# tachitachi/SR-WaveNet

Measured on AMD Instinct MI355X. Metric: audio samples/sec (fwd+bwd) 30-layer teacher WaveNet, higher is better.
Workload: dtype bf16; 1 GPU; 30-layer teacher WaveNet (3x[1..512] dilations, 64 res / 256 skip ch, 256-way mu-law softmax), fwd+bwd+Adam, batch 8x16000 samples per GPU; global_batch=8, seq_len=16000, parallelism=dp1, launch=hipGraph

## Files before the change

sr-wavenet_amd/build.py:

```python
from __future__ import annotations

import os
import subprocess
import sys
from concurrent.futures import ThreadPoolExecutor

HERE = os.path.dirname(os.path.abspath(__file__))
CSRC = os.path.join(HERE, "csrc")
LIB = os.path.join(HERE, "libsrwn.so")
MANIFEST = os.path.join(HERE, "libsrwn.manifest.json")
IO_LIB = os.path.join(HERE, "libsrwn_io.so")
PYB_SRC = os.path.join(CSRC, "srwn_pybind.cpp")
PYB_NAME = "_srwn_pyb"
IO_SOURCES = ["srwn_tfrecord.cpp"]
CXX = os.environ.get("CXX", "g++")
SOURCES = ["srwn_util.hip", "srwn_fwd.hip", "srwn_bwd.hip", "srwn_opt.hip", "srwn_pool.hip", "srwn_gemm.hip", "srwn_wgrad2.hip", "srwn_gen.hip", "srwn_gen16.hip", "srwn_flow.hip", "srwn_enc.hip", "srwn_nc.hip", "srwn_ncstream.hip", "srwn_group.hip", "srwn_wgradt.hip", "srwn_ops.hip", "srwn_head.hip", "srwn_siamese.hip", "srwn_wngate.hip", "srwn_stream.hip", "srwn_recog.hip", "srwn_score.hip", "srwn_embed.hip", "srwn_flow_inv.hip", "srwn_data.hip", "srwn_draw.hip", "srwn_augment.hip", "srwn_resample.hip", "srwn_room.hip", "srwn_eval.hip", "srwn_pair_eval.hip"]
HIPCC = os.environ.get("HIPCC", "/opt/rocm/bin/hipcc")
FLAGS = ["--offload-arch=gfx950", "-O3", "-fPIC", "-std=c++17", "-Wno-pass-failed", "-ffp-contract=on"]
NO_SPILL = {"srwn_wgradt.hip": ["wgrad_skip_wt_kernel"], "srwn_siamese.hip": ["contrastive_head_kernel"],
            "srwn_wngate.hip": ["wavenet_layer_fwd_kernel", "wavenet_layer_bwd_kernel"],
            "srwn_ncstream.hip": ["nc_encode_frames_kernel", "nc_encode_frames_kernelINS_10NcListArgs"],
            "srwn_recog.hip": ["pooled_stream_head_kernel"], "srwn_score.hip": ["stream_score_head_kernel"],
            "srwn_embed.hip": ["window_embed_match_kernel", "gallery_match_kernel"],
            "srwn_pair_eval.hip": ["embed_collect_kernel", "pair_sweep_kernel"],
            "srwn_room.hip": ["batch_draw_room_kernel", "pair_draw_room_kernel"]}


def _deps():
    hdrs = [os.path.join(CSRC, f) for f in os.listdir(CSRC) if f.endswith(".h")]
    hdrs.append(os.path.join(HERE, "..", "include", "srwn.h"))
    return hdrs


def source_hashes():
    import hashlib
    files = [os.path.join(CSRC, f) for f in sorted(os.listdir(CSRC)) if f.endswith((".hip", ".h", ".cpp"))]
    files.append(os.path.join(HERE, "..", "include", "srwn.h"))
    files.append(os.path.join(HERE, "..", "include", "srwn_io.h"))
    out = {}
    for f in files:
        if os.path.exists(f):
            out[os.path.relpath(f, os.path.join(HERE, ".."))] = hashlib.sha256(open(f, "rb").read()).hexdigest()
    return out


def _stale(target, srcs):
    if not os.path.exists(target):
        return True
    t = os.path.getmtime(target)
    return any(os.path.getmtime(s) > t for s in srcs)


def _sha(paths, extra=""):
    import hashlib
    h = hashlib.sha256(extra.encode())
    for f in paths:
        h.update(open(f, "rb").read())
    return h.hexdigest()


def _check_no_spill(src, obj, remarks, kernels):
    import re
    seen = {}
    name = None
    for line in remarks.splitlines():
        m = re.search(r"Function Name: (\S+)", line)
        if m:
            name = m.group(1)
        m = re.search(r"(?:[VS]GPRs Spill|ScratchSize \[bytes/lane\]): (\d+)", line)
        if m and name:
            seen[name] = seen.get(name, 0) + int(m.group(1))
    for k in kernels:
        hit = [(n, v) for n, v in seen.items() if k in n]
        if not hit or any(v for _, v in hit):
            if os.path.exists(obj):
                os.remove(obj)
            raise RuntimeError("%s: kernel %s must not spill registers or use scratch: %s" % (src, k, hit or "not found"))


def _check_inflight(src, obj, flags, kernels):
    import importlib.util
    spec = importlib.util.spec_from_file_location("_srwn_asmcheck", os.path.join(HERE, "asmcheck.py"))
    ac = importlib.util.module_from_spec(spec)
    spec.loader.exec_module(ac)
    cmd = [HIPCC] + flags + ["--cuda-device-only", "-S", src, "-o", "-"]
    r = subprocess.run(cmd, capture_output=True, text=True)
    if r.returncode != 0:
        raise RuntimeError("hipcc -S failed for %s:\n%s" % (src, r.stderr[-4000:]))
    for k in kernels:
        bad = ac.check_inflight_loads(r.stdout, k)
        if bad:
            if os.path.exists(obj):
                os.remove(obj)
            raise RuntimeError("%s: kernel %s touches the destination of a load that may still be in flight:\n  %s"
                               % (src, k, "\n  ".join(bad[:8])))


def build(force: bool = False, verbose: bool = False, diag: bool = False, variant: str = "", extra_flags=()) -> str:
    import json
    per_src = {}
    for f in list(extra_flags):
        if ".hip:" in f:
            name, fl = f.split(":", 1)
            per_src.setdefault(name, []).extend(fl.split("=", 1) if fl.startswith("-mllvm=") else [fl])
    extra_flags = [f for f in extra_flags if ".hip:" not in f]
    flags = FLAGS + (["-DSRWN_DIAG"] if diag else []) + list(extra_flags)
    if variant:
        diag = True
# ... 132 lines not shown
```

sr-wavenet_amd/csrc/srwn_gemm.hip:

```cpp
#include <cstdlib>
#include "srwn_common.h"
#include "srwn_host.h"
#include "../../include/srwn.h"

using namespace srwn;

#define SRWN_EPI_SOFTMAX_CE 3

struct RgArgs {
  const void* x; int64_t x_row_stride; int64_t x_chunk_stride; int chunk_len; int ks_total;
  const void* wpack; const float* bias; void* y; int64_t y_row_stride; int cout_valid; int64_t rows;
  const void* aux; int64_t aux_row_stride;
  const int32_t* targets; float* loss_partials; float* logits_out; float grad_scale;
  int tap_T; int tap_step; const float* frame_add; int64_t frame_add_ld; int frames; int pool; float frame_add_scale;
  int safe_wait;
  unsigned long long* stamps;
};

#ifndef SRWN_RG_PIPE
#define SRWN_RG_PIPE 1
#endif
#ifndef SRWN_RG_PIPE_VALU
#define SRWN_RG_PIPE_VALU 6
#endif
constexpr bool kRgPipe = SRWN_RG_PIPE != 0;
constexpr int kRgPipeValu = SRWN_RG_PIPE_VALU;
template <bool STAMP> struct RgStamper {
  unsigned long long* p; int n;
  __device__ __forceinline__ void operator()(int tag) {
    if (STAMP && p && n < 512) { p[n] = ((unsigned long long)tag << 48) | (__builtin_amdgcn_s_memtime() & 0xffffffffffffull); ++n; }
  }
};

template <typename T> __device__ __forceinline__ void glds16(const void* g, void* l) {
  __builtin_amdgcn_global_load_lds((const __attribute__((address_space(1))) void*)g,
                                   (__attribute__((address_space(3))) void*)l, 16, 0, 0);
}

__device__ __forceinline__ void glds16_untracked(const void* g, unsigned lds_addr) {
  unsigned keep;
  asm volatile("s_mov_b32 %0, m0\n\ts_mov_b32 m0, %2\n\ts_nop 0\n\tglobal_load_lds_dwordx4 %1, off\n\ts_mov_b32 m0, %0"
               : "=&s"(keep) : "v"(g), "s"(lds_addr) : "memory");
}

constexpr int rg_waves(int epi, int nt) { return (epi == SRWN_EPI_SOFTMAX_CE || nt == 2) ? 4 : 8; }

template <typename T, int MT, int KSC, int PRO, int EPI, int NT, bool TAPS = false, bool STAMP = false>
__global__ __launch_bounds__(64 * rg_waves(EPI, NT), (EPI == SRWN_EPI_SOFTMAX_CE || NT == 2) ? 1 : 2) void rowgemm_kernel(RgArgs a) {
  constexpr int kRgWaves = rg_waves(EPI, NT);
  RgStamper<STAMP> stamp{nullptr, 0};
  if (STAMP && blockIdx.x == 0 && (threadIdx.x & 63) == 0 && ((threadIdx.x >> 6) & 3) == 0) stamp.p = a.stamps + (threadIdx.x >> 8) * 512;
  stamp(1);
  static_assert(MT % 2 == 0, "outputs are emitted in 64-channel groups");
  static_assert(EPI != SRWN_EPI_SOFTMAX_CE || NT == 1, "softmax epilogue holds one column tile");
  constexpr int FB = sizeof(Frag<T>) * 64;
  constexpr int CHUNK_B = MT * KSC * FB;
  constexpr int PIECES = CHUNK_B / 1024;
  static_assert(PIECES % kRgWaves == 0, "chunk must split evenly over the waves");
  extern __shared__ __attribute__((aligned(16))) char smem[];

  const int lane = threadIdx.x & 63;
  const int wave = __builtin_amdgcn_readfirstlane(threadIdx.x >> 6);
  const int col = lane & 31, half = lane >> 5;
  const int64_t tile0 = ((int64_t)blockIdx.x * kRgWaves + wave) * NT;
  int64_t rowv[NT];
  bool valid[NT];
  int tclip[NT];
#pragma unroll
  for (int nt = 0; nt < NT; ++nt) {
    rowv[nt] = (tile0 + nt) * 32 + col;
    valid[nt] = rowv[nt] < a.rows;
    tclip[nt] = TAPS ? (int)((valid[nt] ? rowv[nt] : (a.rows - 1)) % a.tap_T) : 0;
  }
  const int nchunks = a.ks_total / KSC;
  const char* wbase = reinterpret_cast<const char*>(a.wpack);
  const unsigned lds_base = (unsigned)(size_t)(__attribute__((address_space(3))) char*)smem;

  auto stage = [&](int c, int buf) {
#pragma unroll
    for (int i = 0; i < PIECES / kRgWaves; ++i) {
      const int p = wave * (PIECES / kRgWaves) + i;
      const int mt = p / (KSC * FB / 1024), within = (p % (KSC * FB / 1024)) * 1024;
      const char* g = wbase + ((size_t)mt * a.ks_total + (size_t)c * KSC) * FB + within + lane * 16;
      const unsigned l = lds_base + (unsigned)(buf * CHUNK_B + mt * (KSC * FB) + within);
      glds16_untracked(g, __builtin_amdgcn_readfirstlane(l));
    }
  };
  int cur_chunk = 0, cur_within = 0, cur_next = 0;
  int64_t cur_off = 0;
  const int64_t chunk_step = a.x_chunk_stride - a.chunk_len + 16;
  auto cursor = [&](int (&chunk)[KSC], int (&within)[KSC], int64_t (&off)[KSC]) {
    int cc = cur_chunk, ww = cur_within;
    int64_t oo = cur_off;
#pragma unroll
    for (int ks = 0; ks < KSC; ++ks) {
      chunk[ks] = cc; within[ks] = ww; off[ks] = oo;
      const bool wrap = ww + 16 >= a.chunk_len;
      ww = wrap ? 0 : ww + 16;
      oo += wrap ? chunk_step : (int64_t)16;
      cc += wrap ? 1 : 0;
    }
    if (cur_next + 1 < nchunks) { cur_chunk = cc; cur_within = ww; cur_off = oo; ++cur_next; }
  };
  auto load_b = [&](Frag<T> (&dst)[NT][KSC], bool (&ok)[NT][KSC]) {
    int chunks[KSC], withins[KSC];
    int64_t offs[KSC];
    cursor(chunks, withins, offs);
#pragma unroll
    for (int nt = 0; nt < NT; ++nt)
#pragma unroll
      for (int ks = 0; ks < KSC; ++ks) {
        const int chunk = chunks[ks], within = withins[ks];
        const int64_t rbase = valid[nt] ? rowv[nt] : (a.rows - 1);
        if (TAPS) {
          const int tp = tclip[nt] + chunk * a.tap_step;
          ok[nt][ks] = tp >= 0 && tp < a.tap_T;
          const T* p = reinterpret_cast<const T*>(a.x) + (rbase + (ok[nt][ks] ? chunk * a.tap_step : 0)) * a.x_row_stride +
                       within + 8 * half;
          dst[nt][ks] = load_nat(p);
        } else {
          ok[nt][ks] = true;
          const T* p = reinterpret_cast<const T*>(a.x) + offs[ks] + rbase * a.x_row_stride + 8 * half;
          dst[nt][ks] = load_nat(p);
        }
      }
// ... 191 lines not shown
    float s = 0.0f;
    {
      const int cv = opaque(a.cout_valid);
#pragma unroll
      for (int mt = 0; mt < MT; ++mt)
#pragma unroll
        for (int q = 0; q < 16; ++q) {
          const int n = 32 * mt + crow(q, half);
          const float e = (n < cv) ? __expf(acc[mt][0][q] - m) : 0.0f;
          acc[mt][0][q] = e;
          s += e;
        }
    }
    s += __shfl_xor(s, 32);
    const float lse = m + __logf(s);
    float loss = (vld && half == 0) ? (lse - vt) : 0.0f;
#pragma unroll
    for (int off = 16; off > 0; off >>= 1) loss += __shfl_xor(loss, off);
    if (lane == 0 && tile0 * 32 < a.rows) a.loss_partials[tile0] = loss;
    if (a.y) {
      const float ps = a.grad_scale / s;
      const int64_t r0 = tile0 * 32;
      const int rows_valid = (a.rows - r0) < 32 ? (int)(a.rows - r0) : 32;
      T* ytile = reinterpret_cast<T*>(a.y) + (rows_valid > 0 ? r0 : 0) * a.y_row_stride;
#pragma unroll
      for (int j = 0; j < MT / 2; ++j) {
        const int tg = opaque(tgt);
        float v[2][16];
#pragma unroll
        for (int m2 = 0; m2 < 2; ++m2)
#pragma unroll
          for (int q = 0; q < 16; ++q) {
            const int n = 32 * (2 * j + m2) + crow(q, half);
            v[m2][q] = fmaf(acc[2 * j + m2][0][q], ps, n == tg ? -a.grad_scale : 0.0f);
          }
        store_rows_via_lds<T, 2>(rstage, ytile + 64 * j, a.y_row_stride, v, rows_valid, lane);
      }
    }
    return;
  }

#pragma unroll
  for (int nt = 0; nt < NT; ++nt) {
    const int64_t r0 = (tile0 + nt) * 32;
    const int rows_valid = (a.rows - r0) < 32 ? (int)(a.rows - r0) : 32;
    T* ytile = reinterpret_cast<T*>(a.y) + (rows_valid > 0 ? r0 : 0) * a.y_row_stride;
    const T* arow = (EPI == SRWN_EPI_MASK)
                        ? reinterpret_cast<const T*>(a.aux) + (valid[nt] ? rowv[nt] : 0) * a.aux_row_stride
                        : nullptr;
    const float* frow = nullptr;
    if (TAPS && a.frame_add) {
      const int64_t rr = valid[nt] ? rowv[nt] : 0;
      frow = a.frame_add + ((rr / a.tap_T) * a.frames + (tclip[nt] / a.pool)) * a.frame_add_ld;
    }
#pragma unroll
    for (int j = 0; j < MT / 2; ++j) {
      if (64 * j >= a.cout_valid) continue;
      float v[2][16];
#pragma unroll
      for (int m2 = 0; m2 < 2; ++m2)
#pragma unroll
        for (int g = 0; g < 4; ++g) {
          f32x4 mk = {1.f, 1.f, 1.f, 1.f};
          if (EPI == SRWN_EPI_MASK) mk = load4(arow + 32 * (2 * j + m2) + 8 * g + 4 * half);
          f32x4 fa = {0.f, 0.f, 0.f, 0.f};
          if (TAPS && frow) fa = *reinterpret_cast<const f32x4*>(frow + 32 * (2 * j + m2) + 8 * g + 4 * half);
#pragma unroll
          for (int e = 0; e < 4; ++e) {
            float x = acc[2 * j + m2][nt][4 * g + e];
            if (TAPS) x = fmaf(fa[e], a.frame_add_scale, x);
            if (EPI == SRWN_EPI_RELU) x = fmaxf(x, 0.0f);
            if (EPI == SRWN_EPI_MASK) x = (mk[e] > 0.0f) ? x : 0.0f;
            v[m2][4 * g + e] = x;
          }
        }
      store_rows_via_lds<T, 2>(rstage, ytile + 64 * j, a.y_row_stride, v, rows_valid, lane);
    }
  }
}

struct CgArgs {
  const void* x; int64_t x_row_stride; const void* wpack; void* y; int64_t y_layer_stride; int nlayers; int64_t rows;
  int safe_wait;
};

template <typename T, int RT, int KSS, int NBUF, int NW>
__global__ __launch_bounds__(64 * NW) void colgemm_kernel(CgArgs a) {
  constexpr int R = 32 * RT;
  constexpr int FB = sizeof(Frag<T>) * 64;
  constexpr int CHUNK_B = RT * KSS * FB;
  extern __shared__ __attribute__((aligned(16))) char smem[];
  const int lane = threadIdx.x & 63;
  const int wave = __builtin_amdgcn_readfirstlane(threadIdx.x >> 6);
  const int col = lane & 31, half = lane >> 5;
  T* stage = reinterpret_cast<T*>(smem + NBUF * CHUNK_B) + wave * (32 * RowStage<T>::stride(R));
  const int64_t row0 = ((int64_t)blockIdx.x * NW + wave) * 32;
  const int64_t row = row0 + col;
  const bool valid = row < a.rows;
  const int rows_valid = (a.rows - row0) < 32 ? (int)(a.rows - row0) : 32;
  const char* wbase = reinterpret_cast<const char*>(a.wpack);

  constexpr bool COUNTED = sizeof(T) == 2 && NBUF == 2;
  constexpr int PIECES = CHUNK_B / 1024;
  static_assert(!COUNTED || PIECES % NW == 0, "weight image must split evenly over the waves");
  const unsigned lds_base = (unsigned)(size_t)(__attribute__((address_space(3))) char*)smem;
  auto dma = [&](int l, int buf) __attribute__((always_inline)) {
#pragma unroll
    for (int i = 0; i < PIECES / NW; ++i) {
      const int p = wave * (PIECES / NW) + i;
      glds16_untracked(wbase + (size_t)l * CHUNK_B + (size_t)p * 1024 + lane * 16,
                       __builtin_amdgcn_readfirstlane(lds_base + (unsigned)(buf * CHUNK_B + p * 1024)));
    }
  };
  if constexpr (COUNTED) dma(0, 0); else lds_dma_copy(wbase, smem, CHUNK_B, wave, lane, NW);
  Frag<T> bf[KSS];
  {
    const T* p = reinterpret_cast<const T*>(a.x) + (valid ? row : 0) * a.x_row_stride + 8 * half;
#pragma unroll
    for (int ks = 0; ks < KSS; ++ks) bf[ks] = load_nat(p + 16 * ks);
#pragma unroll
    for (int ks = 0; ks < KSS; ++ks) bf[ks] = valid ? bf[ks] : zero_frag<T>();
  }
  if constexpr (COUNTED) asm volatile("s_waitcnt vmcnt(0)" ::: "memory");
  __syncthreads();
  for (int l = 0; l < a.nlayers; ++l) {
    const int buf = (NBUF == 2) ? (l & 1) : 0;
    if (NBUF == 2 && l + 1 < a.nlayers) {
      if constexpr (COUNTED) dma(l + 1, (l + 1) & 1);
      else lds_dma_copy(wbase + (size_t)(l + 1) * CHUNK_B, smem + ((l + 1) & 1) * CHUNK_B, CHUNK_B, wave, lane, NW);
    }
    const Frag<T>* lw = reinterpret_cast<const Frag<T>*>(smem + buf * CHUNK_B) + lane;
    f32x16 acc[RT];
#pragma unroll
    for (int mt = 0; mt < RT; ++mt)
#pragma unroll
      for (int q = 0; q < 16; ++q) acc[mt][q] = 0.0f;
    constexpr int G = 4;
    Frag<T> af[2][G][RT];
#pragma unroll
    for (int j = 0; j < G; ++j)
#pragma unroll
      for (int mt = 0; mt < RT; ++mt) af[0][j][mt] = lw[(mt * KSS + j) * 64];
#pragma unroll
    for (int k0 = 0; k0 < KSS; k0 += G) {
      if (k0 + G < KSS) {
#pragma unroll
        for (int j = 0; j < G; ++j)
#pragma unroll
          for (int mt = 0; mt < RT; ++mt) af[((k0 / G) + 1) & 1][j][mt] = lw[(mt * KSS + k0 + G + j) * 64];
      }
      __builtin_amdgcn_sched_barrier(0);
#pragma unroll
      for (int j = 0; j < G; ++j)
#pragma unroll
        for (int mt = 0; mt < RT; ++mt) mma(acc[mt], af[(k0 / G) & 1][j][mt], bf[k0 + j]);
      __builtin_amdgcn_sched_barrier(0);
    }
    float v[RT][16];
#pragma unroll
    for (int mt = 0; mt < RT; ++mt)
#pragma unroll
      for (int q = 0; q < 16; ++q) v[mt][q] = acc[mt][q];
    T* ytile = reinterpret_cast<T*>(a.y) + (int64_t)l * a.y_layer_stride + (rows_valid > 0 ? row0 : 0) * R;
    if constexpr (COUNTED) {
      constexpr int STORES = 32 / (64 / (R / RowStage<T>::VEC));
      if (rows_valid > 0) {
        store_rows_via_lds<T, RT, true>(stage, ytile, R, v, rows_valid, lane);
        if (a.safe_wait) asm volatile("s_waitcnt vmcnt(0)" ::: "memory");
        else asm volatile("s_waitcnt vmcnt(%0)" ::"n"(STORES) : "memory");
      } else {
        asm volatile("s_waitcnt vmcnt(0)" ::: "memory");
      }
      asm volatile("s_waitcnt lgkmcnt(0)\n\ts_barrier" ::: "memory");
    } else {
      store_rows_via_lds<T, RT>(stage, ytile, R, v, rows_valid, lane);
      __syncthreads();
    }
    if (NBUF == 1 && l + 1 < a.nlayers) {
      lds_dma_copy(wbase + (size_t)(l + 1) * CHUNK_B, smem, CHUNK_B, wave, lane, NW);
      __syncthreads();
    }
  }
}

template <typename T, int RT, int KSS, int NBUF>
static int launch_cg(const CgArgs& a, hipStream_t st) {
  constexpr int R = 32 * RT;
  constexpr int NW = (sizeof(T) == 2) ? 8 : 4;
  const size_t sh = (size_t)NBUF * RT * KSS * sizeof(Frag<T>) * 64 + (size_t)NW * 32 * RowStage<T>::stride(R) * sizeof(T);
  auto kfn = colgemm_kernel<T, RT, KSS, NBUF, NW>;
  hipError_t e = hipFuncSetAttribute((const void*)kfn, hipFuncAttributeMaxDynamicSharedMemorySize, (int)sh);
  if (e != hipSuccess) return set_error((int)e, "skip_dgrad_all: LDS %zu: %s", sh, hipGetErrorString(e));
  hipLaunchKernelGGL(kfn, dim3((unsigned)((a.rows + 32 * NW - 1) / (32 * NW))), dim3(64 * NW), sh, st, a);
  return check_launch("skip_dgrad_all");
}

extern "C" int srwn_skip_dgrad_all(const void* dtotal, const void* wskipT_all, void* dcs, int64_t dcs_layer_stride,
                                   int32_t nlayers, int64_t rows, int32_t R, int32_t S, int32_t dtype, void* stream) {
  if (rows == 0 || nlayers == 0) return 0;
  if (!dtotal || !wskipT_all || !dcs) return set_error(SRWN_E_NULL, "skip_dgrad_all: null pointer");
  if (rows < 0 || nlayers < 0) return set_error(SRWN_E_SHAPE, "skip_dgrad_all: rows=%lld layers=%d", (long long)rows, nlayers);
  CgArgs a{dtotal, S, wskipT_all, dcs, dcs_layer_stride, nlayers, rows, safe_wait()};
  hipStream_t st = (hipStream_t)stream;
  if (R == 64 && S == 256) {
    if (dtype == SRWN_BF16) return launch_cg<bf16_t, 2, 16, 2>(a, st);
    if (dtype == SRWN_F32) return launch_cg<float, 2, 16, 1>(a, st);
    return set_error(SRWN_E_DTYPE, "skip_dgrad_all: dtype %d", dtype);
  }
  if (R == 32 && S == 128) {
    if (dtype == SRWN_BF16) return launch_cg<bf16_t, 1, 8, 2>(a, st);
    if (dtype == SRWN_F32) return launch_cg<float, 1, 8, 2>(a, st);
    return set_error(SRWN_E_DTYPE, "skip_dgrad_all: dtype %d", dtype);
  }
  return set_error(SRWN_E_UNSUPPORTED, "skip_dgrad_all: built for (R,S) = (64,256) and (32,128), got (%d,%d)", R, S);
}

namespace srwn {

template <typename T, int MT, int KSC, int NT>
static int launch_rg(const RgArgs& a, int pro, int epi, hipStream_t st) {
  constexpr int CHUNK_B = MT * KSC * (int)sizeof(Frag<T>) * 64;
  constexpr int NTS = 1;
  const int nw = rg_waves(epi, (epi == SRWN_EPI_SOFTMAX_CE) ? NTS : NT);
  const size_t stage_b = (size_t)nw * 32 * RowStage<T>::stride(64) * sizeof(T);
  const size_t sh = 2 * (size_t)CHUNK_B > stage_b ? 2 * (size_t)CHUNK_B : stage_b;
  const int rows_per_block = 32 * nw * ((epi == SRWN_EPI_SOFTMAX_CE) ? NTS : NT);
  dim3 grid((unsigned)((a.rows + rows_per_block - 1) / rows_per_block)), block(64 * nw);
#define SRWN_RG(P, E)                                                                                        \
  if (pro == P && epi == E) {                                                                                \
    auto kfn = rowgemm_kernel<T, MT, KSC, P, E, (E == SRWN_EPI_SOFTMAX_CE) ? 1 : NT>;                        \
    if constexpr (sizeof(T) == 2 && P == SRWN_PRO_GATE && E == SRWN_EPI_RELU && NT == 1 && MT == 8) {         \
      SRWN_DIAG_ONLY(if (a.stamps) kfn = rowgemm_kernel<T, MT, KSC, P, E, NT, false, true>;)    \
    }                                                                                                        \
    if (sh > 32768) {                                                                                        \
      hipError_t e = hipFuncSetAttribute((const void*)kfn, hipFuncAttributeMaxDynamicSharedMemorySize, (int)sh); \
      if (e != hipSuccess) return set_error((int)e, "rowgemm: LDS %zu: %s", sh, hipGetErrorString(e));       \
    }                                                                                                        \
    hipLaunchKernelGGL(kfn, grid, block, sh, st, a);                                                         \
    return check_launch("rowgemm");                                                                          \
  }
  SRWN_RG(SRWN_PRO_NONE, SRWN_EPI_NONE)
  SRWN_RG(SRWN_PRO_NONE, SRWN_EPI_RELU)
  SRWN_RG(SRWN_PRO_NONE, SRWN_EPI_MASK)
  SRWN_RG(SRWN_PRO_GATE, SRWN_EPI_NONE)
  SRWN_RG(SRWN_PRO_GATE, SRWN_EPI_RELU)
  SRWN_RG(SRWN_PRO_NONE, SRWN_EPI_SOFTMAX_CE)
#undef SRWN_RG
  return set_error(SRWN_E_UNSUPPORTED, "rowgemm: pro %d / epi %d combination not built", pro, epi);
}

template <typename T, int MT, int KSC>
static int launch_rg_taps(const RgArgs& a, int epi, hipStream_t st) {
  constexpr int CHUNK_B = MT * KSC * (int)sizeof(Frag<T>) * 64;
  constexpr int kRgWaves = rg_waves(SRWN_EPI_NONE, 1);
  const size_t stage_b = (size_t)kRgWaves * 32 * RowStage<T>::stride(64) * sizeof(T);
  const size_t sh = 2 * (size_t)CHUNK_B > stage_b ? 2 * (size_t)CHUNK_B : stage_b;
  dim3 grid((unsigned)((a.rows + 32 * kRgWaves - 1) / (32 * kRgWaves))), block(64 * kRgWaves);
#define SRWN_RGT(E)                                                                                          \
  if (epi == E) {                                                                                            \
    auto kfn = rowgemm_kernel<T, MT, KSC, SRWN_PRO_NONE, E, 1, true>;                                        \
    if (sh > 32768) {                                                                                        \
      hipError_t e = hipFuncSetAttribute((const void*)kfn, hipFuncAttributeMaxDynamicSharedMemorySize, (int)sh); \
      if (e != hipSuccess) return set_error((int)e, "tap_linear: LDS %zu: %s", sh, hipGetErrorString(e));    \
    }                                                                                                        \
    hipLaunchKernelGGL(kfn, grid, block, sh, st, a);                                                         \
    return check_launch("tap_linear");                                                                       \
  }
  SRWN_RGT(SRWN_EPI_NONE)
  SRWN_RGT(SRWN_EPI_RELU)
  SRWN_RGT(SRWN_EPI_MASK)
#undef SRWN_RGT
  return set_error(SRWN_E_UNSUPPORTED, "tap_linear: epilogue %d not built", epi);
}

int rowgemm_dispatch(const void* x, int64_t x_row_stride, int64_t x_chunk_stride, int chunk_len, int Cin,
                     const void* wpack, const float* bias, void* y, int64_t y_row_stride, int cout_pad,
                     int cout_valid, int64_t rows, const void* aux, int64_t aux_row_stride, const int32_t* targets,
                     float* loss_partials, float* logits_out, float grad_scale, int pro, int epi, int dtype,
                     hipStream_t st, int* rc) {
  if ((cout_pad != 256 && cout_pad != 128) || (Cin % 64) != 0 || rows < 1 || chunk_len < 16 || (chunk_len % 16) != 0) return 0;
  if (epi != SRWN_EPI_SOFTMAX_CE && (cout_valid % 64) != 0) return 0;
  if (cout_pad == 128) {
    if (epi == SRWN_EPI_SOFTMAX_CE) return 0;
    RgArgs a4{x, x_row_stride, x_chunk_stride, chunk_len, Cin / 16, wpack, bias, y, y_row_stride, cout_valid, rows,
              aux, aux_row_stride, targets, loss_partials, logits_out, grad_scale, 0, 0, nullptr, 0, 0, 1, 0.0f, safe_wait(), nullptr};
// ... 37 lines not shown
```

sr-wavenet_amd/csrc/srwn_head.hip:

```cpp
#include <cstdlib>
#include "srwn_common.h"
#include "srwn_host.h"
#include "../../include/srwn.h"

using namespace srwn;

namespace {

__device__ __forceinline__ void glds16_untracked(const void* g, unsigned lds_addr) {
  unsigned keep;
  asm volatile("s_mov_b32 %0, m0\n\ts_mov_b32 m0, %2\n\ts_nop 0\n\tglobal_load_lds_dwordx4 %1, off\n\ts_mov_b32 m0, %0"
               : "=&s"(keep) : "v"(g), "s"(lds_addr) : "memory");
}

typedef unsigned u32x2 __attribute__((ext_vector_type(2)));
typedef unsigned u32x4 __attribute__((ext_vector_type(4)));
typedef float f32x2_t __attribute__((ext_vector_type(2)));
typedef __bf16 bf16x2_t __attribute__((ext_vector_type(2)));
__device__ __forceinline__ unsigned pack2(float lo, float hi) {
  return __builtin_bit_cast(unsigned, __builtin_convertvector(f32x2_t{lo, hi}, bf16x2_t));
}

typedef short i16x2_t __attribute__((ext_vector_type(2)));
typedef unsigned short u16x2_t __attribute__((ext_vector_type(2)));
__device__ __forceinline__ unsigned pk_relu(unsigned w) {
  return __builtin_bit_cast(unsigned, __builtin_elementwise_max(__builtin_bit_cast(i16x2_t, w), i16x2_t{0, 0}));
}
__device__ __forceinline__ unsigned pk_nonzero(unsigned w) {
  unsigned d;
  asm("v_pk_min_u16 %0, %1, %2" : "=v"(d) : "v"(w), "s"(0x00010001u));
  return d;
}
__device__ __forceinline__ unsigned pk_ones(unsigned b) {
  unsigned d;
  asm("v_pk_mul_lo_u16 %0, %1, %2" : "=v"(d) : "v"(b), "s"(0xffffffffu));
  return d;
}

struct HcArgs {
  const void* r0;
  const void* w[4];
  const float* b1; const float* b2;
  const int32_t* targets; float* loss_partials; float grad_scale; int cout_valid;
  void* r1; void* dlogits; void* da1; void* dtotal;
  int64_t rows;
  unsigned long long* stamps;
  int safe_wait;
  int stagger;
  int first_round;
};

constexpr int kHcWaves = 8;
constexpr int kHcBufs = 3;
template <int V> struct IC { static constexpr int value = V; };

template <bool STAMP> struct HcStamper {
  unsigned long long* p; int n;
  __device__ __forceinline__ void operator()(int tag) {
    if (STAMP && p && n < 512) { p[n] = ((unsigned long long)tag << 48) | (__builtin_amdgcn_s_memtime() & 0xffffffffffffull); ++n; }
  }
};

template <typename T, bool STAMP = false>
__global__ __launch_bounds__(64 * kHcWaves) void headchain_kernel(HcArgs a) {
  constexpr int MT = 8, KS = 16, KSC = 4, NCH = KS / KSC, C = 256;
  constexpr int FB = (int)sizeof(Frag<T>) * 64, CHUNK_B = MT * KSC * FB, PIECES = CHUNK_B / 1024;
  static_assert(PIECES % kHcWaves == 0, "chunk must split evenly over the waves");
  extern __shared__ __attribute__((aligned(16))) char smem[];
  const int lane = threadIdx.x & 63;
  const int wave = __builtin_amdgcn_readfirstlane(threadIdx.x >> 6);
  const int col = lane & 31, half = lane >> 5;
  const int64_t tile = (int64_t)blockIdx.x * kHcWaves + wave;
  const int64_t r0row = tile * 32;
  const int64_t row = r0row + col;
  const bool valid = row < a.rows;
  const int64_t rowc = valid ? row : (a.rows - 1);
  const int rows_valid = (a.rows - r0row) < 32 ? (int)(a.rows - r0row) : 32;
  T* rstage = reinterpret_cast<T*>(smem + kHcBufs * CHUNK_B) + wave * (32 * RowStage<T>::stride(64));
  float* lbias = reinterpret_cast<float*>(smem + kHcBufs * CHUNK_B + kHcWaves * 32 * RowStage<T>::stride(64) * sizeof(T));
  unsigned char* gbits = reinterpret_cast<unsigned char*>(lbias + 2 * C) + wave * (32 * 33);
  for (int i = threadIdx.x; i < 2 * C; i += 64 * kHcWaves) lbias[i] = i < C ? a.b1[i] : (i - C < a.cout_valid ? a.b2[i - C] : -1e30f);
  const unsigned lds_base = (unsigned)(size_t)(__attribute__((address_space(3))) char*)smem;
  HcStamper<STAMP> stamp{nullptr, 0};
  if (STAMP && blockIdx.x == 0 && lane == 0 && wave < 2) stamp.p = a.stamps + wave * 512;
  stamp(1);
  if (a.stagger > 0 && (int)blockIdx.x < a.first_round) {
    const int d = (int)((blockIdx.x >> 3) & 7) * a.stagger;
    for (int i = 0; i < d; ++i) __builtin_amdgcn_s_sleep(16);
  }

  auto stage = [&](int g, int buf) __attribute__((always_inline)) {
    const char* wbase = reinterpret_cast<const char*>(a.w[g / NCH]);
    const int c = g % NCH;
#pragma unroll
    for (int i = 0; i < PIECES / kHcWaves; ++i) {
      const int p = wave * (PIECES / kHcWaves) + i;
      const int mt = p / (KSC * FB / 1024), within = (p % (KSC * FB / 1024)) * 1024;
      const char* gsrc = wbase + ((size_t)mt * KS + (size_t)c * KSC) * FB + within + lane * 16;
      glds16_untracked(gsrc, __builtin_amdgcn_readfirstlane(lds_base + (unsigned)(buf * CHUNK_B + mt * (KSC * FB) + within)));
    }
  };

  const int tgt = valid ? a.targets[row] : -1;
  Frag<T> bfr[KS];
  stage(0, 0);
  if (kHcBufs > 2) stage(1, 1);
  {
    const T* xr = reinterpret_cast<const T*>(a.r0) + rowc * C + 8 * half;
#pragma unroll
    for (int ks = 0; ks < KS; ++ks) bfr[ks] = load_nat(xr + 16 * ks);
  }
#pragma unroll
  for (int ks = 0; ks < KS; ++ks) {
    const u32x4 wd = __builtin_bit_cast(u32x4, bfr[ks].v);
    unsigned b = 0u;
#pragma unroll
    for (int e = 3; e >= 0; --e) b = (b << 2) | pk_nonzero(pk_relu(wd[e]));
    gbits[col * 33 + 2 * ks + half] = (unsigned char)(b | (b >> 15));
  }
  f32x16 acc[MT];
  unsigned m1[4] = {0u, 0u, 0u, 0u};
  asm volatile("s_waitcnt vmcnt(0)" ::: "memory");
  __syncthreads();
  stamp(2);
  auto cn = [](int mt, int q) { return 32 * mt + crow(q, 0); };
  auto seed = [&](int mt, const float* nb) __attribute__((always_inline)) {
#pragma unroll
    for (int g = 0; g < 4; ++g) {
      const f32x4 b = nb ? *reinterpret_cast<const f32x4*>(nb + 4 * half + 32 * mt + 8 * g) : f32x4{0.f, 0.f, 0.f, 0.f};
#pragma unroll
      for (int r = 0; r < 4; ++r) acc[mt][4 * g + r] = b[r];
    }
  };
#pragma unroll
  for (int mt = 0; mt < MT; ++mt) seed(mt, lbias);

  auto finish = [&](void* dst, auto fn, bool gated, const float* nextbias, bool frags) __attribute__((always_inline)) {
    constexpr int LS = RowStage<T>::stride(64);
    T* ytile = reinterpret_cast<T*>(dst) + (rows_valid > 0 ? r0row : 0) * C;
    const int rsub = lane >> 3, piece = lane & 7;
    const int rv = __builtin_amdgcn_readfirstlane(rows_valid);
#pragma unroll
    for (int j = 0; j < MT / 2; ++j) {
      unsigned pk[2][8];
#pragma unroll
      for (int m2 = 0; m2 < 2; ++m2)
#pragma unroll
        for (int i = 0; i < 8; ++i)
          pk[m2][i] = fn(j, 8 * m2 + i, acc[2 * j + m2][2 * i], acc[2 * j + m2][2 * i + 1]);
      wave_lds_order();
#pragma unroll
      for (int m2 = 0; m2 < 2; ++m2)
#pragma unroll
        for (int g = 0; g < 4; ++g)
          *reinterpret_cast<u32x2*>(rstage + col * LS + 32 * m2 + 8 * g + 4 * half) = u32x2{pk[m2][2 * g], pk[m2][2 * g + 1]};
      wave_lds_order();
#pragma unroll
      for (int i = 0; i < 4; ++i) {
        const int r = min(8 * i + rsub, rv - 1);
        u32x4 v = *reinterpret_cast<const u32x4*>(rstage + r * LS + piece * 8);
        if (gated) {
          const int b = gbits[max(r, 0) * 33 + 8 * j + piece];
#pragma unroll
          for (int e = 0; e < 4; ++e)
            v[e] &= __builtin_amdgcn_perm((unsigned)__builtin_amdgcn_sbfe(b, 2 * e + 1, 1), (unsigned)__builtin_amdgcn_sbfe(b, 2 * e, 1), 0x05040100u);
        }
        if (rv > 0) __builtin_nontemporal_store(v, reinterpret_cast<u32x4*>(ytile + r * C + 64 * j + piece * 8));
      }
      if (frags) {
#pragma unroll
        for (int m2 = 0; m2 < 2; ++m2)
#pragma unroll
          for (int h2 = 0; h2 < 2; ++h2) {
            const u32x4 w{pk[m2][4 * h2], pk[m2][4 * h2 + 1], pk[m2][4 * h2 + 2], pk[m2][4 * h2 + 3]};
            bfr[2 * (2 * j + m2) + h2].v = __builtin_bit_cast(bf16x8, w);
          }
      }
      seed(2 * j, nextbias);
      seed(2 * j + 1, nextbias);
      __builtin_amdgcn_sched_barrier(0);
    }
  };

  auto step = [&](auto gc) __attribute__((always_inline)) {
    constexpr int g = decltype(gc)::value;
// ... 1 lines not shown
    constexpr int AHEAD = kHcBufs - 1;
    if (g + AHEAD < 4 * NCH) stage(g + AHEAD, (g + AHEAD) % kHcBufs);
    stamp(10);
    const Frag<T>* lw = reinterpret_cast<const Frag<T>*>(smem + (g % kHcBufs) * CHUNK_B) + lane;
    {
      constexpr int NF = KSC * MT;
      Frag<T> af[3];
      af[0] = lw[0];
      af[1] = lw[(1 * KSC) * 64];
#pragma unroll
      for (int f = 0; f < NF; ++f) {
        const int ks = f / MT, mt = f % MT;
        if (f + 2 < NF) af[(f + 2) % 3] = lw[(((f + 2) % MT) * KSC + (f + 2) / MT) * 64];
        __builtin_amdgcn_sched_barrier(0);
        mma(acc[mt], af[f % 3], bfr[c * KSC + ks]);
      }
    }
    stamp(11);
    if constexpr (AHEAD > 1 && g + AHEAD < 4 * NCH) {
      if (a.safe_wait) asm volatile("s_waitcnt vmcnt(0)" ::: "memory");
      else asm volatile("s_waitcnt vmcnt(%0)" ::"n"(PIECES / kHcWaves) : "memory");
    }
    else asm volatile("s_waitcnt vmcnt(0)" ::: "memory");
    stamp(12);
    if constexpr (c == NCH - 1) {
      if constexpr (s == 0) {
        finish(a.r1, [&](int j, int idx, float a0, float a1) {
          const unsigned w = pk_relu(pack2(a0, a1));
          m1[j] = (m1[j] << 1) | pk_nonzero(w);
          asm volatile("" : "+v"(m1[j]));
          return w; }, false, lbias + C, true);
      } else if constexpr (s == 1) {
        auto opaque = [](int x) { asm volatile("" : "+v"(x)); return x; };
        const int tgh = opaque(tgt - 4 * half);
        float m = -INFINITY, vt = 0.0f;
#pragma unroll
        for (int mt = 0; mt < MT; ++mt)
#pragma unroll
          for (int q = 0; q < 16; q += 2) {
            m = fmaxf(fmaxf(m, acc[mt][q]), acc[mt][q + 1]);
            vt = cn(mt, q) == tgh ? acc[mt][q] : vt;
            vt = cn(mt, q + 1) == tgh ? acc[mt][q + 1] : vt;
          }
        m = fmaxf(m, __shfl_xor(m, 32));
        vt += __shfl_xor(vt, 32);
        const float ml = -m * 1.4426950408889634f;
        float sum = 0.0f;
#pragma unroll
        for (int mt = 0; mt < MT; ++mt)
#pragma unroll
          for (int q = 0; q < 16; ++q) {
            acc[mt][q] = __builtin_amdgcn_exp2f(fmaf(acc[mt][q], 1.4426950408889634f, ml));
            sum += acc[mt][q];
          }
        sum += __shfl_xor(sum, 32);
        const float lse = m + __logf(sum);
        float loss = (valid && half == 0) ? (lse - vt) : 0.0f;
#pragma unroll
        for (int off = 16; off > 0; off >>= 1) loss += __shfl_xor(loss, off);
        if (lane == 0 && rows_valid > 0) a.loss_partials[tile] = loss;
        const float ps = a.grad_scale / sum, ngs = -a.grad_scale;
        const int tgc = opaque(tgt - 4 * half);
        finish(a.dlogits, [&](int j, int idx, float a0, float a1) {
          const int n = cn(2 * j + (idx >> 3), 2 * (idx & 7));
          return pack2(fmaf(a0, ps, n == tgc ? ngs : 0.0f), fmaf(a1, ps, n + 1 == tgc ? ngs : 0.0f)); }, false, nullptr, true);
      } else if constexpr (s == 2) {
        finish(a.da1, [&](int j, int idx, float a0, float a1) {
          const unsigned k0 = (unsigned)__builtin_amdgcn_sbfe((int)m1[j], 15 - idx, 1);
          const unsigned k1 = (unsigned)__builtin_amdgcn_sbfe((int)m1[j], 31 - idx, 1);
          return pack2(__uint_as_float(__float_as_uint(a0) & k0), __uint_as_float(__float_as_uint(a1) & k1)); },
               false, nullptr, true);
      } else {
        finish(a.dtotal, [&](int j, int idx, float a0, float a1) { return pack2(a0, a1); }, true, nullptr, false);
      }
    }
    if constexpr (c == NCH - 1) stamp(13);
    __syncthreads();
    stamp(14);
  };
  step(IC<0>{});  step(IC<1>{});  step(IC<2>{});  step(IC<3>{});
  step(IC<4>{});  step(IC<5>{});  step(IC<6>{});  step(IC<7>{});
  step(IC<8>{});  step(IC<9>{});  step(IC<10>{}); step(IC<11>{});
  step(IC<12>{}); step(IC<13>{}); step(IC<14>{}); step(IC<15>{});
}

}

static int num_cus_hc() {
  static int cus = 0;
  if (cus == 0) {
    int dev = 0, n = 0;
    cus = (hipGetDevice(&dev) == hipSuccess && hipDeviceGetAttribute(&n, hipDeviceAttributeMultiprocessorCount, dev) == hipSuccess && n > 0) ? n : 256;
  }
  return cus;
}

extern "C" int srwn_head_chain(const void* r0, const void* w1, const void* w2_perm, const void* w2T_perm,
                               const void* w1T_perm, const float* b1, const float* b2, const int32_t* targets,
                               float* loss_partials, void* r1, void* dlogits, void* da1, void* dtotal, int32_t S,
                               int32_t cout_pad, int32_t cout_valid, int64_t rows, float grad_scale, int32_t dtype,
                               void* stream) {
  if (rows == 0) return 0;
  if (!r0 || !w1 || !w2_perm || !w2T_perm || !w1T_perm || !b1 || !b2 || !targets || !loss_partials || !r1 ||
      !dlogits || !da1 || !dtotal)
    return set_error(SRWN_E_NULL, "head_chain: null pointer");
  if (dtype != SRWN_BF16) return set_error(SRWN_E_UNSUPPORTED, "head_chain: built for bf16 (fp32 keeps the four launches)");
  if (S != 256 || cout_pad != 256) return set_error(SRWN_E_UNSUPPORTED, "head_chain: built for 256 skip channels and <= 256 classes (S=%d, cout_pad=%d)", S, cout_pad);
  if (rows < 0 || cout_valid < 1 || cout_valid > 256 || (rows + 31) / 32 / kHcWaves + 1 > 0x7fffffffLL)
    return set_error(SRWN_E_SHAPE, "head_chain: rows=%lld cout_valid=%d", (long long)rows, cout_valid);
  HcArgs a{r0, {w1, w2_perm, w2T_perm, w1T_perm}, b1, b2, targets, loss_partials, grad_scale, cout_valid,
           r1, dlogits, da1, dtotal, rows, debug_stamps(), safe_wait(), 0, 0};
  {
    static const int stg = [] { const char* e = getenv("SRWN_HC_STAGGER"); return e ? atoi(e) : 2; }();
    a.stagger = stg;
    a.first_round = num_cus_hc();
  }
  const int64_t tiles = (rows + 31) / 32;
  const size_t sh = kHcBufs * (size_t)(8 * 4 * 1024) + (size_t)kHcWaves * 32 * RowStage<bf16_t>::stride(64) * sizeof(bf16_t) + 2 * 256 * sizeof(float) + (size_t)kHcWaves * 32 * 33;
  auto kfn = headchain_kernel<bf16_t, false>;
  SRWN_DIAG_ONLY(if (a.stamps) kfn = headchain_kernel<bf16_t, true>;)
  hipError_t e = hipFuncSetAttribute((const void*)kfn, hipFuncAttributeMaxDynamicSharedMemorySize, (int)sh);
  if (e != hipSuccess) return set_error((int)e, "head_chain: LDS %zu: %s", sh, hipGetErrorString(e));
  hipLaunchKernelGGL(kfn, dim3((unsigned)((tiles + kHcWaves - 1) / kHcWaves)), dim3(64 * kHcWaves), sh,
                     (hipStream_t)stream, a);
  return check_launch("head_chain");
}
```

sr-wavenet_amd/csrc/srwn_host.h:

```cpp
#pragma once
#include <cstdarg>
#include <cstdio>
#include <cstdint>
#include <hip/hip_runtime.h>

namespace srwn {
int set_error(int code, const char* fmt, ...);
int check_launch(const char* what);
int rowgemm_dispatch(const void* x, int64_t x_row_stride, int64_t x_chunk_stride, int chunk_len, int Cin,
                     const void* wpack, const float* bias, void* y, int64_t y_row_stride, int cout_pad,
                     int cout_valid, int64_t rows, const void* aux, int64_t aux_row_stride, const int32_t* targets,
                     float* loss_partials, float* logits_out, float grad_scale, int pro, int epi, int dtype,
                     hipStream_t st, int* rc);
unsigned long long* debug_stamps();
#ifdef SRWN_DIAG
#define SRWN_DIAG_ONLY(...) __VA_ARGS__
#else
#define SRWN_DIAG_ONLY(...)
#endif
int safe_wait();
}
```

Measured before the change: 79.52 million samples/s.

## Make colgemm and head-chain kernels persistent with cross-tile weight and input prefetch

Result: no change. 79.51 million samples/s (median of 2 runs) (-0.0%).

```diff
diff --git a/sr-wavenet_amd/build.py b/sr-wavenet_amd/build.py
--- a/sr-wavenet_amd/build.py
+++ b/sr-wavenet_amd/build.py
@@ -23,7 +23,8 @@
             "srwn_recog.hip": ["pooled_stream_head_kernel"], "srwn_score.hip": ["stream_score_head_kernel"],
             "srwn_embed.hip": ["window_embed_match_kernel", "gallery_match_kernel"],
             "srwn_pair_eval.hip": ["embed_collect_kernel", "pair_sweep_kernel"],
-            "srwn_room.hip": ["batch_draw_room_kernel", "pair_draw_room_kernel"]}
+            "srwn_room.hip": ["batch_draw_room_kernel", "pair_draw_room_kernel"],
+            "srwn_head.hip": ["headchain_kernel"], "srwn_gemm.hip": ["colgemm_kernel"]}
 
 
 def _deps():
diff --git a/sr-wavenet_amd/csrc/srwn_gemm.hip b/sr-wavenet_amd/csrc/srwn_gemm.hip
--- a/sr-wavenet_amd/csrc/srwn_gemm.hip
+++ b/sr-wavenet_amd/csrc/srwn_gemm.hip
@@ -41,6 +41,12 @@
   unsigned keep;
   asm volatile("s_mov_b32 %0, m0\n\ts_mov_b32 m0, %2\n\ts_nop 0\n\tglobal_load_lds_dwordx4 %1, off\n\ts_mov_b32 m0, %0"
                : "=&s"(keep) : "v"(g), "s"(lds_addr) : "memory");
+}
+
+__device__ __forceinline__ void glds16_untracked_s(const void* sbase, unsigned voff, unsigned lds_addr) {
+  unsigned keep;
+  asm volatile("s_mov_b32 %0, m0\n\ts_mov_b32 m0, %3\n\ts_nop 0\n\tglobal_load_lds_dwordx4 %1, %2\n\ts_mov_b32 m0, %0"
+               : "=&s"(keep) : "v"(voff), "s"(sbase), "s"(lds_addr) : "memory");
 }
 
 constexpr int rg_waves(int epi, int nt) { return (epi == SRWN_EPI_SOFTMAX_CE || nt == 2) ? 4 : 8; }
@@ -398,9 +404,12 @@
 struct CgArgs {
   const void* x; int64_t x_row_stride; const void* wpack; void* y; int64_t y_layer_stride; int nlayers; int64_t rows;
   int safe_wait;
+  int blocks;
 };
 
-template <typename T, int RT, int KSS, int NBUF, int NW>
+template <bool V> struct CgFlag { static constexpr bool value = V; };
+
+template <typename T, int RT, int KSS, int NBUF, int NW, bool ONE = false>
 __global__ __launch_bounds__(64 * NW) void colgemm_kernel(CgArgs a) {
   constexpr int R = 32 * RT;
   constexpr int FB = sizeof(Frag<T>) * 64;
@@ -410,41 +419,33 @@
   const int wave = __builtin_amdgcn_readfirstlane(threadIdx.x >> 6);
   const int col = lane & 31, half = lane >> 5;
   T* stage = reinterpret_cast<T*>(smem + NBUF * CHUNK_B) + wave * (32 * RowStage<T>::stride(R));
-  const int64_t row0 = ((int64_t)blockIdx.x * NW + wave) * 32;
-  const int64_t row = row0 + col;
-  const bool valid = row < a.rows;
-  const int rows_valid = (a.rows - row0) < 32 ? (int)(a.rows - row0) : 32;
   const char* wbase = reinterpret_cast<const char*>(a.wpack);
+  const int nblk = a.blocks, nl = a.nlayers;
 
   constexpr bool COUNTED = sizeof(T) == 2 && NBUF == 2;
   constexpr int PIECES = CHUNK_B / 1024;
   static_assert(!COUNTED || PIECES % NW == 0, "weight image must split evenly over the waves");
   const unsigned lds_base = (unsigned)(size_t)(__attribute__((address_space(3))) char*)smem;
+  const unsigned lane16 = (unsigned)lane * 16u;
   auto dma = [&](int l, int buf) __attribute__((always_inline)) {
 #pragma unroll
     for (int i = 0; i < PIECES / NW; ++i) {
       const int p = wave * (PIECES / NW) + i;
-      glds16_untracked(wbase + (size_t)l * CHUNK_B + (size_t)p * 1024 + lane * 16,
-                       __builtin_amdgcn_readfirstlane(lds_base + (unsigned)(buf * CHUNK_B + p * 1024)));
+      glds16_untracked_s(wbase + (size_t)l * CHUNK_B + (size_t)p * 1024, lane16,
+                         __builtin_amdgcn_readfirstlane(lds_base + (unsigned)(buf * CHUNK_B + p * 1024)));
     }
   };
-  if constexpr (COUNTED) dma(0, 0); else lds_dma_copy(wbase, smem, CHUNK_B, wave, lane, NW);
+  auto xrow = [&](int blk) __attribute__((always_inline)) {
+    const int64_t r = ((int64_t)blk * NW + wave) * 32 + col;
+    return reinterpret_cast<const T*>(a.x) + (r < a.rows ? r : 0) * a.x_row_stride + 8 * half;
+  };
+  int64_t row0 = 0;
+  int rows_valid = 0;
+  bool valid = false;
   Frag<T> bf[KSS];
-  {
-    const T* p = reinterpret_cast<const T*>(a.x) + (valid ? row : 0) * a.x_row_stride + 8 * half;
-#pragma unroll
-    for (int ks = 0; ks < KSS; ++ks) bf[ks] = load_nat(p + 16 * ks);
-#pragma unroll
-    for (int ks = 0; ks < KSS; ++ks) bf[ks] = valid ? bf[ks] : zero_frag<T>();
-  }
-  if constexpr (COUNTED) asm volatile("s_waitcnt vmcnt(0)" ::: "memory");
-  __syncthreads();
-  for (int l = 0; l < a.nlayers; ++l) {
-    const int buf = (NBUF == 2) ? (l & 1) : 0;
-    if (NBUF == 2 && l + 1 < a.nlayers) {
-      if constexpr (COUNTED) dma(l + 1, (l + 1) & 1);
-      else lds_dma_copy(wbase + (size_t)(l + 1) * CHUNK_B, smem + ((l + 1) & 1) * CHUNK_B, CHUNK_B, wave, lane, NW);
-    }
+
+  auto layer = [&](int l, int buf, auto refill_c, const T* xn) __attribute__((always_inline)) {
+    constexpr bool REFILL = decltype(refill_c)::value;
     const Frag<T>* lw = reinterpret_cast<const Frag<T>*>(smem + buf * CHUNK_B) + lane;
     f32x16 acc[RT];
 #pragma unroll
@@ -471,6 +472,11 @@
 #pragma unroll
         for (int mt = 0; mt < RT; ++mt) mma(acc[mt], af[(k0 / G) & 1][j][mt], bf[k0 + j]);
       __builtin_amdgcn_sched_barrier(0);
+      if constexpr (REFILL) {
+#pragma unroll
+        for (int j = 0; j < G; ++j) bf[k0 + j] = load_nat(xn + 16 * (k0 + j));
+        __builtin_amdgcn_sched_barrier(0);
+      }
     }
     float v[RT][16];
 #pragma unroll
@@ -483,7 +489,7 @@
       if (rows_valid > 0) {
         store_rows_via_lds<T, RT, true>(stage, ytile, R, v, rows_valid, lane);
         if (a.safe_wait) asm volatile("s_waitcnt vmcnt(0)" ::: "memory");
-        else asm volatile("s_waitcnt vmcnt(%0)" ::"n"(STORES) : "memory");
+        else asm volatile("s_waitcnt vmcnt(%0)" ::"n"(STORES + (REFILL ? KSS : 0)) : "memory");
       } else {
         asm volatile("s_waitcnt vmcnt(0)" ::: "memory");
       }
@@ -492,22 +498,89 @@
       store_rows_via_lds<T, RT>(stage, ytile, R, v, rows_valid, lane);
       __syncthreads();
     }
-    if (NBUF == 1 && l + 1 < a.nlayers) {
-      lds_dma_copy(wbase + (size_t)(l + 1) * CHUNK_B, smem, CHUNK_B, wave, lane, NW);
+  };
+
+  using No = CgFlag<false>;
+  using Yes = CgFlag<true>;
+  int blk = blockIdx.x;
+  int g = 0;
+  if constexpr (COUNTED) {
+    dma(0, 0);
+    const T* p = xrow(blk);
+#pragma unroll
+    for (int ks = 0; ks < KSS; ++ks) bf[ks] = load_nat(p + 16 * ks);
+    if (a.safe_wait) asm volatile("s_waitcnt vmcnt(0)" ::: "memory");
+    else asm volatile("s_waitcnt vmcnt(%0)" ::"n"(KSS) : "memory");
+    asm volatile("s_waitcnt lgkmcnt(0)\n\ts_barrier" ::: "memory");
+  }
+  for (; blk < nblk; blk += (int)gridDim.x) {
+    row0 = ((int64_t)blk * NW + wave) * 32;
+    valid = row0 + col < a.rows;
+    rows_valid = (a.rows - row0) < 32 ? (int)(a.rows - row0) : 32;
+    if constexpr (COUNTED) {
+      const int nxt = blk + (int)gridDim.x;
+      const bool more = nxt < nblk;
+      const T* xn = xrow(more ? nxt : blk);
+      if constexpr (ONE) {
+        if (more) {
+          dma(0, (g + 1) & 1);
+          layer(0, g & 1, Yes{}, xn);
+        } else {
+          layer(0, g & 1, No{}, xn);
+        }
+        ++g;
+      } else {
+        dma(1, (g + 1) & 1);
+        layer(0, g & 1, No{}, xn);
+        ++g;
+        const int plain = more ? nl - 1 : nl;
+        for (int l = 1; l < plain; ++l, ++g) {
+          if (l + 1 < nl) dma(l + 1, (g + 1) & 1);
+          layer(l, g & 1, No{}, xn);
+        }
+        if (more) {
+          dma(0, (g + 1) & 1);
+          layer(nl - 1, g & 1, Yes{}, xn);
+          ++g;
+        }
+      }
+    } else {
+      lds_dma_copy(wbase, smem, CHUNK_B, wave, lane, NW);
+      const T* p = xrow(blk);
+#pragma unroll
+      for (int ks = 0; ks < KSS; ++ks) bf[ks] = load_nat(p + 16 * ks);
+#pragma unroll
+      for (int ks = 0; ks < KSS; ++ks) bf[ks] = valid ? bf[ks] : zero_frag<T>();
       __syncthreads();
+      for (int l = 0; l < nl; ++l) {
+        if (NBUF == 2 && l + 1 < nl)
+          lds_dma_copy(wbase + (size_t)(l + 1) * CHUNK_B, smem + ((l + 1) & 1) * CHUNK_B, CHUNK_B, wave, lane, NW);
+        layer(l, (NBUF == 2) ? (l & 1) : 0, No{}, p);
+        if (NBUF == 1 && l + 1 < nl) {
+          lds_dma_copy(wbase + (size_t)(l + 1) * CHUNK_B, smem, CHUNK_B, wave, lane, NW);
+          __syncthreads();
+        }
+      }
     }
   }
 }
 
 template <typename T, int RT, int KSS, int NBUF>
-static int launch_cg(const CgArgs& a, hipStream_t st) {
+static int launch_cg(CgArgs a, hipStream_t st) {
   constexpr int R = 32 * RT;
   constexpr int NW = (sizeof(T) == 2) ? 8 : 4;
   const size_t sh = (size_t)NBUF * RT * KSS * sizeof(Frag<T>) * 64 + (size_t)NW * 32 * RowStage<T>::stride(R) * sizeof(T);
   auto kfn = colgemm_kernel<T, RT, KSS, NBUF, NW>;
+  if constexpr (sizeof(T) == 2 && NBUF == 2) {
+    if (a.nlayers == 1) kfn = colgemm_kernel<T, RT, KSS, NBUF, NW, true>;
+  }
   hipError_t e = hipFuncSetAttribute((const void*)kfn, hipFuncAttributeMaxDynamicSharedMemorySize, (int)sh);
   if (e != hipSuccess) return set_error((int)e, "skip_dgrad_all: LDS %zu: %s", sh, hipGetErrorString(e));
-  hipLaunchKernelGGL(kfn, dim3((unsigned)((a.rows + 32 * NW - 1) / (32 * NW))), dim3(64 * NW), sh, st, a);
+  const int64_t blocks = (a.rows + 32 * NW - 1) / (32 * NW);
+  if (blocks > 0x7fffffffLL) return set_error(SRWN_E_SHAPE, "skip_dgrad_all: rows=%lld", (long long)a.rows);
+  a.blocks = (int)blocks;
+  const int grid = gemm_grid();
+  hipLaunchKernelGGL(kfn, dim3((unsigned)(blocks < grid ? blocks : grid)), dim3(64 * NW), sh, st, a);
   return check_launch("skip_dgrad_all");
 }
 
@@ -516,7 +589,7 @@
   if (rows == 0 || nlayers == 0) return 0;
   if (!dtotal || !wskipT_all || !dcs) return set_error(SRWN_E_NULL, "skip_dgrad_all: null pointer");
   if (rows < 0 || nlayers < 0) return set_error(SRWN_E_SHAPE, "skip_dgrad_all: rows=%lld layers=%d", (long long)rows, nlayers);
-  CgArgs a{dtotal, S, wskipT_all, dcs, dcs_layer_stride, nlayers, rows, safe_wait()};
+  CgArgs a{dtotal, S, wskipT_all, dcs, dcs_layer_stride, nlayers, rows, safe_wait(), 0};
   hipStream_t st = (hipStream_t)stream;
   if (R == 64 && S == 256) {
     if (dtype == SRWN_BF16) return launch_cg<bf16_t, 2, 16, 2>(a, st);
diff --git a/sr-wavenet_amd/csrc/srwn_head.hip b/sr-wavenet_amd/csrc/srwn_head.hip
--- a/sr-wavenet_amd/csrc/srwn_head.hip
+++ b/sr-wavenet_amd/csrc/srwn_head.hip
@@ -7,10 +7,10 @@
 
 namespace {
 
-__device__ __forceinline__ void glds16_untracked(const void* g, unsigned lds_addr) {
+__device__ __forceinline__ void glds16_untracked_s(const void* sbase, unsigned voff, unsigned lds_addr) {
   unsigned keep;
-  asm volatile("s_mov_b32 %0, m0\n\ts_mov_b32 m0, %2\n\ts_nop 0\n\tglobal_load_lds_dwordx4 %1, off\n\ts_mov_b32 m0, %0"
-               : "=&s"(keep) : "v"(g), "s"(lds_addr) : "memory");
+  asm volatile("s_mov_b32 %0, m0\n\ts_mov_b32 m0, %3\n\ts_nop 0\n\tglobal_load_lds_dwordx4 %1, %2\n\ts_mov_b32 m0, %0"
+               : "=&s"(keep) : "v"(voff), "s"(sbase), "s"(lds_addr) : "memory");
 }
 
 typedef unsigned u32x2 __attribute__((ext_vector_type(2)));
@@ -48,6 +48,7 @@
   int safe_wait;
   int stagger;
   int first_round;
+  int blocks;
 };
 
 constexpr int kHcWaves = 8;
@@ -67,40 +68,47 @@
   constexpr int FB = (int)sizeof(Frag<T>) * 64, CHUNK_B = MT * KSC * FB, PIECES = CHUNK_B / 1024;
   static_assert(PIECES % kHcWaves == 0, "chunk must split evenly over the waves");
   extern __shared__ __attribute__((aligned(16))) char smem[];
-  const int lane = threadIdx.x & 63;
+  const int lane0 = threadIdx.x & 63;
   const int wave = __builtin_amdgcn_readfirstlane(threadIdx.x >> 6);
+  T* rstage = reinterpret_cast<T*>(smem + kHcBufs * CHUNK_B) + wave * (32 * RowStage<T>::stride(64));
+  float* lbias = reinterpret_cast<float*>(smem + kHcBufs * CHUNK_B + kHcWaves * 32 * RowStage<T>::stride(64) * sizeof(T));
+  unsigned char* gbits_w = reinterpret_cast<unsigned char*>(lbias + 2 * C) + wave * (32 * 33);
+  for (int i = threadIdx.x; i < 2 * C; i += 64 * kHcWaves) lbias[i] = i < C ? a.b1[i] : (i - C < a.cout_valid ? a.b2[i - C] : -1e30f);
+  const unsigned lds_base = (unsigned)(size_t)(__attribute__((address_space(3))) char*)smem;
+  unsigned lane16 = 0u;
+  HcStamper<STAMP> stamp{nullptr, 0};
+  if (STAMP && blockIdx.x == 0 && lane0 == 0 && wave < 2) stamp.p = a.stamps + wave * 512;
+  stamp(1);
+  if (a.stagger > 0 && (int)blockIdx.x < a.first_round) {
+    const int d = (int)((blockIdx.x >> 3) & 7) * a.stagger;
+    for (int i = 0; i < d; ++i) __builtin_amdgcn_s_sleep(16);
+  }
+
+  auto stage = [&](int g, int buf) __attribute__((always_inline)) {
+    const char* wbase = reinterpret_cast<const char*>(a.w[g / NCH]);
+    asm volatile("" : "+s"(wbase));
+    const int c = g % NCH;
+#pragma unroll
+    for (int i = 0; i < PIECES / kHcWaves; ++i) {
+      const int p = wave * (PIECES / kHcWaves) + i;
+      const int mt = p / (KSC * FB / 1024), within = (p % (KSC * FB / 1024)) * 1024;
+      glds16_untracked_s(wbase + ((size_t)mt * KS + (size_t)c * KSC) * FB + within, lane16,
+                         __builtin_amdgcn_readfirstlane(lds_base + (unsigned)(buf * CHUNK_B + mt * (KSC * FB) + within)));
+    }
+  };
+
+  for (int blk = blockIdx.x; blk < a.blocks; blk += (int)gridDim.x) {
+  int lane = lane0;
+  asm volatile("" : "+v"(lane));
   const int col = lane & 31, half = lane >> 5;
-  const int64_t tile = (int64_t)blockIdx.x * kHcWaves + wave;
+  lane16 = (unsigned)lane * 16u;
+  unsigned char* gbits = gbits_w;
+  const int64_t tile = (int64_t)blk * kHcWaves + wave;
   const int64_t r0row = tile * 32;
   const int64_t row = r0row + col;
   const bool valid = row < a.rows;
   const int64_t rowc = valid ? row : (a.rows - 1);
   const int rows_valid = (a.rows - r0row) < 32 ? (int)(a.rows - r0row) : 32;
-  T* rstage = reinterpret_cast<T*>(smem + kHcBufs * CHUNK_B) + wave * (32 * RowStage<T>::stride(64));
-  float* lbias = reinterpret_cast<float*>(smem + kHcBufs * CHUNK_B + kHcWaves * 32 * RowStage<T>::stride(64) * sizeof(T));
-  unsigned char* gbits = reinterpret_cast<unsigned char*>(lbias + 2 * C) + wave * (32 * 33);
-  for (int i = threadIdx.x; i < 2 * C; i += 64 * kHcWaves) lbias[i] = i < C ? a.b1[i] : (i - C < a.cout_valid ? a.b2[i - C] : -1e30f);
-  const unsigned lds_base = (unsigned)(size_t)(__attribute__((address_space(3))) char*)smem;
-  HcStamper<STAMP> stamp{nullptr, 0};
-  if (STAMP && blockIdx.x == 0 && lane == 0 && wave < 2) stamp.p = a.stamps + wave * 512;
-  stamp(1);
-  if (a.stagger > 0 && (int)blockIdx.x < a.first_round) {
-    const int d = (int)((blockIdx.x >> 3) & 7) * a.stagger;
-    for (int i = 0; i < d; ++i) __builtin_amdgcn_s_sleep(16);
-  }
-
-  auto stage = [&](int g, int buf) __attribute__((always_inline)) {
-    const char* wbase = reinterpret_cast<const char*>(a.w[g / NCH]);
-    const int c = g % NCH;
-#pragma unroll
-    for (int i = 0; i < PIECES / kHcWaves; ++i) {
-      const int p = wave * (PIECES / kHcWaves) + i;
-      const int mt = p / (KSC * FB / 1024), within = (p % (KSC * FB / 1024)) * 1024;
-      const char* gsrc = wbase + ((size_t)mt * KS + (size_t)c * KSC) * FB + within + lane * 16;
-      glds16_untracked(gsrc, __builtin_amdgcn_readfirstlane(lds_base + (unsigned)(buf * CHUNK_B + mt * (KSC * FB) + within)));
-    }
-  };
-
   const int tgt = valid ? a.targets[row] : -1;
   Frag<T> bfr[KS];
   stage(0, 0);
@@ -268,6 +276,7 @@
   step(IC<4>{});  step(IC<5>{});  step(IC<6>{});  step(IC<7>{});
   step(IC<8>{});  step(IC<9>{});  step(IC<10>{}); step(IC<11>{});
   step(IC<12>{}); step(IC<13>{}); step(IC<14>{}); step(IC<15>{});
+  }
 }
 
 }
@@ -295,7 +304,7 @@
   if (rows < 0 || cout_valid < 1 || cout_valid > 256 || (rows + 31) / 32 / kHcWaves + 1 > 0x7fffffffLL)
     return set_error(SRWN_E_SHAPE, "head_chain: rows=%lld cout_valid=%d", (long long)rows, cout_valid);
   HcArgs a{r0, {w1, w2_perm, w2T_perm, w1T_perm}, b1, b2, targets, loss_partials, grad_scale, cout_valid,
-           r1, dlogits, da1, dtotal, rows, debug_stamps(), safe_wait(), 0, 0};
+           r1, dlogits, da1, dtotal, rows, debug_stamps(), safe_wait(), 0, 0, 0};
   {
     static const int stg = [] { const char* e = getenv("SRWN_HC_STAGGER"); return e ? atoi(e) : 2; }();
     a.stagger = stg;
@@ -307,7 +316,10 @@
   SRWN_DIAG_ONLY(if (a.stamps) kfn = headchain_kernel<bf16_t, true>;)
   hipError_t e = hipFuncSetAttribute((const void*)kfn, hipFuncAttributeMaxDynamicSharedMemorySize, (int)sh);
   if (e != hipSuccess) return set_error((int)e, "head_chain: LDS %zu: %s", sh, hipGetErrorString(e));
-  hipLaunchKernelGGL(kfn, dim3((unsigned)((tiles + kHcWaves - 1) / kHcWaves)), dim3(64 * kHcWaves), sh,
+  const int64_t blocks = (tiles + kHcWaves - 1) / kHcWaves;
+  const int grid = gemm_grid();
+  a.blocks = (int)blocks;
+  hipLaunchKernelGGL(kfn, dim3((unsigned)(blocks < grid ? blocks : grid)), dim3(64 * kHcWaves), sh,
                      (hipStream_t)stream, a);
   return check_launch("head_chain");
 }
diff --git a/sr-wavenet_amd/csrc/srwn_host.h b/sr-wavenet_amd/csrc/srwn_host.h
--- a/sr-wavenet_amd/csrc/srwn_host.h
+++ b/sr-wavenet_amd/csrc/srwn_host.h
@@ -2,6 +2,7 @@
 #include <cstdarg>
 #include <cstdio>
 #include <cstdint>
+#include <cstdlib>
 #include <hip/hip_runtime.h>
 
 namespace srwn {
@@ -19,4 +20,14 @@
 #define SRWN_DIAG_ONLY(...)
 #endif
 int safe_wait();
+inline int gemm_grid() {
+  static int cus = 0;
+  if (cus == 0) {
+    int dev = 0, n = 0;
+    cus = (hipGetDevice(&dev) == hipSuccess && hipDeviceGetAttribute(&n, hipDeviceAttributeMultiprocessorCount, dev) == hipSuccess && n > 0) ? n : 256;
+  }
+  const char* e = getenv("SRWN_GEMM_GRID");
+  const long cap = e ? strtol(e, nullptr, 10) : 0;
+  return (cap > 0 && cap < cus) ? (int)cap : cus;
 }
+}
```
